# coroa/tmhpvsim

Hardware: AMD Instinct MI355X
Metric: simulated chain-seconds/sec (node) at 1/2/4/8 GPUs + % HBM roofline (higher is better)
Workload: dtype fp32

## Files before the change

### tmhpvsim_amd/csrc/tmh_engine.hip

```cpp
#include <hip/hip_runtime.h>

#include <algorithm>
#include <climits>
#include <cmath>
#include <cstdarg>
#include <cstdio>
#include <cstdlib>
#include <cstring>
#include <string>
#include <type_traits>
#include <utility>
#include <vector>

#include "tmh_math.h"
#include "tmh_model.h"
#include "tmhpvsim.h"

using namespace tmh;
static_assert(OUT_ANY == TMH_OUT_ANY && OUT_TRACE3 == TMH_OUT_TRACE3 && OUT_STATS == TMH_OUT_STATS &&
                  OUT_SERIES == TMH_OUT_SERIES && OUT_INTERVALS == TMH_OUT_INTERVALS &&
                  OUT_REGISTERS == TMH_OUT_REGISTERS && OUT_DEMAND == TMH_OUT_DEMAND && OUT_STORAGE == TMH_OUT_STORAGE,
              "expansion variants: tmh_model.h and include/tmhpvsim.h agree");

namespace {
// ... 101 lines not shown
    ch.pos = st.pos[c];
    ch.status = st.status[c];
    ch.ncalls = st.ncalls[c];
    ch.t1 = ceil_thr(ch.cl);
    ch.t2 = ceil_thr(ch.cl + ch.clr);
}

__device__ __forceinline__ void store_chain(const StateView& st, uint32_t c, const Chain& ch)
{
#pragma unroll
    for (int k = 0; k < 6; ++k) {
        st.sb[k][c] = ch.s.b[k];
        st.sa[k][c] = ch.s.a[k];
    }
    st.cl[c] = ch.cl;
    st.clr[c] = ch.clr;
    st.mstate[c] = ch.mstate;
    st.sec[c] = ch.sec;
    st.L[c] = ch.L;
    st.pos[c] = ch.pos;
    st.status[c] = ch.status;
    st.ncalls[c] = ch.ncalls;
}

constexpr int INIT_SLOT = CAP - 12;

__device__ __forceinline__ void init_cc_pair(const KParams& kp, uint32_t c, const double* u, double& b, double& a)
{
    Chain ch;
    ch.mstate = 1.0;
    b = draw_cc(kp, gid(kp.ids, c), ch, u[0]);
    a = draw_cc(kp, gid(kp.ids, c), ch, u[1]);
}

__global__ __launch_bounds__(256, BUILD_WAVES) void init_variates_kernel(KParams kp, StateView st, uint64_t chain0, uint32_t n,
                                                            double hf)
{
    const uint32_t c = blockIdx.x * blockDim.x + threadIdx.x;
    const int j = 2 + (int)blockIdx.y;
    if (c >= n) return;
    const uint64_t chain = chain0 + gid(kp.ids, c);
    const U4 blk = keyed_block(kp.seed, chain, 0, TAG_INIT, (uint32_t)(j >> 1));
    const double u = (j & 1) ? u52(blk.z, blk.w) : u52(blk.x, blk.y);
    double v;
    if (j <= 3) {
        v = normal(u, 0.99, 0.08);
    } else if (j >= 10) {
        v = 2.14 * gammaincinv(2.69, u);
    } else {
        const U4 b0 = keyed_block(kp.seed, chain, 0, TAG_INIT, 0);
        const double u01[2] = {u52(b0.x, b0.y), u52(b0.z, b0.w)};
        double ccb, cca;
        init_cc_pair(kp, c, u01, ccb, cca);
        const double cc = interp(ccb, cca, hf);
        if (j <= 5) {
            v = cc < 6.0 / 8 ? normal(u, 0.6784, 0.2046) : (cc < 7.0 / 8 ? NAN : gammaincinv(3.5624, u) * 0.0867 + 0.0);
        } else {
            v = j <= 7 ? scaled_noise(kp, u, 0.01, 0.003, cc) : scaled_noise(kp, u, 0.001, 0.0015, cc);
        }
    }
    sig_c(st, c)[INIT_SLOT + j] = v;
}

template <int RNG>
__global__ __launch_bounds__(256, BUILD_WAVES) void init_kernel(KParams kp, StateView st, uint64_t chain0, uint32_t n,
                                                   double hf, InjView inj)
{
    const uint32_t c = blockIdx.x * blockDim.x + threadIdx.x;
    if (c >= n) return;
    Chain ch;
    for (int k = 0; k < 6; ++k) ch.s.b[k] = ch.s.a[k] = NAN;
    ch.cl = ch.clr = NAN;
    ch.mstate = 1.0;
    ch.sec = 0;
    ch.L = 0;
    ch.t1 = ch.t2 = 0;
    ch.pos = 0;
    ch.status = 0;
    ch.ncalls = 0;
    Draw<RNG> dr;
    if constexpr (RNG == TMH_RNG_KEYED) {
        dr.seed = kp.seed;
        dr.chain = chain0 + gid(kp.ids, c);
    } else {
        dr.u = inj.u + (size_t)c * inj.stride;
        dr.len = inj.len;
    }
    const double* pre = sig_c(st, c) + INIT_SLOT;
    double u[12];
    if constexpr (RNG == TMH_RNG_KEYED) {
        dr.two(ch, 0, TAG_INIT, 0, u[0], u[1]);
    } else {
        for (int d = 0; d < 12; d += 2) dr.two(ch, 0, TAG_INIT, (uint32_t)(d >> 1), u[d], u[d + 1]);
    }
    ch.s.b[S_CC] = draw_cc(kp, gid(kp.ids, c), ch, u[0]);
    ch.s.a[S_CC] = draw_cc(kp, gid(kp.ids, c), ch, u[1]);
    if constexpr (RNG == TMH_RNG_KEYED) {
        ch.s.b[S_CLEAR_DAY] = pre[2];
        ch.s.a[S_CLEAR_DAY] = pre[3];
    } else {
        ch.s.b[S_CLEAR_DAY] = normal(u[2], 0.99, 0.08);
        ch.s.a[S_CLEAR_DAY] = normal(u[3], 0.99, 0.08);
    }
    bool name_error = false;
    for (int j = 0; j < 2; ++j) {
        const double cc = interp(ch.s.b[S_CC], ch.s.a[S_CC], hf);
        double v;
        if (cc < 6.0 / 8) v = RNG == TMH_RNG_KEYED ? pre[4 + j] : normal(u[4 + j], 0.6784, 0.2046);
        else if (cc < 7.0 / 8) {
            name_error = true;
            break;
        } else v = RNG == TMH_RNG_KEYED ? pre[4 + j] : gammaincinv(3.5624, u[4 + j]) * 0.0867 + 0.0;
        if (j == 0) ch.s.b[S_CLOUDY_HOUR] = v;
        else ch.s.a[S_CLOUDY_HOUR] = v;
    }
    if (name_error) {
        if constexpr (RNG == TMH_RNG_INJECTED) ch.pos = ch.pos < 4 ? ch.pos : 4;
        ch.status = TMH_CHAIN_NAMEERROR_INIT;
        store_chain(st, c, ch);
        return;
    }
    if constexpr (RNG == TMH_RNG_KEYED) {
        ch.s.b[S_CLOUDY_NOISE] = pre[6];
        ch.s.a[S_CLOUDY_NOISE] = pre[7];
        ch.s.b[S_CLEAR_NOISE] = pre[8];
        ch.s.a[S_CLEAR_NOISE] = pre[9];
        ch.s.b[S_WS] = pre[10];
        ch.s.a[S_WS] = pre[11];
    } else {
        const double cch = interp(ch.s.b[S_CC], ch.s.a[S_CC], hf);
        ch.s.b[S_CLOUDY_NOISE] = scaled_noise(kp, u[6], 0.01, 0.003, cch);
        ch.s.a[S_CLOUDY_NOISE] = scaled_noise(kp, u[7], 0.01, 0.003, cch);
        ch.s.b[S_CLEAR_NOISE] = scaled_noise(kp, u[8], 0.001, 0.0015, cch);
        ch.s.a[S_CLEAR_NOISE] = scaled_noise(kp, u[9], 0.001, 0.0015, cch);
        ch.s.b[S_WS] = 2.14 * gammaincinv(2.69, u[10]);
        ch.s.a[S_WS] = 2.14 * gammaincinv(2.69, u[11]);
    }
    const double h0 = interp(ch.s.b[S_CC], ch.s.a[S_CC], 0.0);
    const double h = 0.95 < h0 ? 0.95 : h0;
    const double ws = interp(ch.s.b[S_WS], ch.s.a[S_WS], 0.0);
    double* sc = sig_c(st, c);
    double* sl = sig_l(st, c);
    const uint32_t f = next_cloud_fresh<RNG>(kp, sc, sl, ch, dr, h, ws, TAG_INIT_CLOUD);
    if (!f) {
        const double us = dr.one(ch, 0, TAG_INIT_SEC, 0, 0);
        ch.sec = (int32_t)((ch.cl + ch.clr) * us);
    }
    if (f && !ch.status) ch.status = f;
    store_chain(st, c, ch);
    st.fn[0][c] = make_float2((float)ch.s.b[S_CLOUDY_NOISE], (float)ch.s.a[S_CLOUDY_NOISE]);
    st.fn[1][c] = make_float2((float)ch.s.b[S_CLEAR_NOISE], (float)ch.s.a[S_CLEAR_NOISE]);
}

__global__ __launch_bounds__(256, BUILD_WAVES) void geom_kernel(GParams gp, int64_t step0, uint32_t n, double* tab64,
                                                   float* tab32, double* sun)
{
    const uint32_t j = blockIdx.x * blockDim.x + threadIdx.x;
    if (j >= n) return;
    const tmh_clock& ck = gp.clock;
    const int64_t s = step0 + j;
    const int64_t lt = local_at(ck, s), lp = local_at(ck, s > 0 ? s - 1 : 0);
    const int64_t dn = floordiv(lt, 86400), dp = floordiv(lp, 86400);
    const int64_t sod = lt - dn * 86400, sodp = lp - dp * 86400;
    const int hour = (int)(sod / 3600), minute = (int)((sod / 60) % 60), second = (int)(sod % 60);
    const int hourp = (int)(sodp / 3600), minutep = (int)((sodp / 60) % 60);
    double g[ROW];
    for (int i = 0; i < ROW; ++i) g[i] = 0.0;
    clock_fractions(hour, minute, second, g[G_MINF], g[G_HOURF], g[G_DAYF]);
    uint32_t fl = 0;
    if (dn != dp) fl |= FL_DAY;
    if (hour != hourp) fl |= FL_HOUR;
    if (minute != minutep) fl |= FL_MIN;
    int doy, leap;
    civil_doy(dn, doy, leap);
    double sn[SUN_W];
    sun_at(ck.utc0 + s, doy, leap, gp.linke, sn);
    {
        const uint32_t jb = j / BLOCK_STEPS * BLOCK_STEPS;
        double sb[SUN_W];
        if (jb == j) {
            sb[SUN_MIN] = sn[SUN_MIN];
            sb[SUN_EOT] = sn[SUN_EOT];
        } else {
            const int64_t ltb = local_at(ck, step0 + jb);
            int doyb, leapb;
            civil_doy(floordiv(ltb, 86400), doyb, leapb);
            sun_at(ck.utc0 + step0 + jb, doyb, leapb, nullptr, sb);
        }
        const double dh = rad(((sn[SUN_MIN] + sn[SUN_EOT]) - (sb[SUN_MIN] + sb[SUN_EOT])) / 4.0);
        sincos(dh, &sn[SUN_SDH], &sn[SUN_CDH]);
    }
    for (int i = 0; i < SUN_W; ++i) sun[(size_t)j * SUN_W + i] = sn[i];
    site_geom<true>(site_k(gp.site), sn, sn[SUN_TL], gp.module, g);
    if (g[G_GHICS] == 0.0) fl |= FL_NIGHT;
    if (g[G_DISCOK] != 0.0) fl |= FL_DISCOK;
    g[G_FLAGS] = (double)fl;
    double* o64 = tab64 + (size_t)j * ROW;
    for (int i = 0; i < ROW; ++i) o64[i] = g[i];
    table_row32(g, fl, tab32 + (size_t)j * ROW32);
}

__global__ __launch_bounds__(256) void group_kind_kernel(int64_t step0, uint32_t n, float* tab32, double* tab64)
{
    static_assert(BLOCK_STEPS == 128, "a block's 32 groups are the 32 lanes of a half-wave");
    const uint32_t g = blockIdx.x * blockDim.x + threadIdx.x, j = 4 * g;
    uint32_t f[4] = {0u, 0u, 0u, 0u}, k = 0;
    if ((step0 & 3) == 0 && j + 3 < n) {
        uint32_t ev = 0, all = ~0u;
#pragma unroll
        for (int q = 0; q < 4; ++q) {
            f[q] = __float_as_uint(tab32[(size_t)(j + q) * ROW32 + G_FLAGS + G32]);
            all &= f[q];
            if (q > 0) ev |= f[q] & (FL_DAY | FL_HOUR | FL_MIN);
        }
        const uint32_t anyn = (f[0] | f[1] | f[2] | f[3]) & FL_NIGHT;
        if (!ev && (all & FL_NIGHT)) k = FL_G_NIGHT;
        else if (!ev && !anyn && (all & FL_DISCOK)) k = FL_G_DAY;
    }
    const uint64_t ng = __builtin_amdgcn_ballot_w64(k == FL_G_NIGHT);
    const uint32_t half = (threadIdx.x & 32u) ? (uint32_t)(ng >> 32) : (uint32_t)ng;
    if ((threadIdx.x & 31u) == 0 && half == ~0u) k |= FL_B_NIGHT;
    if (k) {
        tab32[(size_t)j * ROW32 + G_FLAGS + G32] = __uint_as_float(f[0] | k);
        tab64[(size_t)j * ROW + G_FLAGS] = (double)(f[0] | k);
    }
}

__global__ __launch_bounds__(1024) void block_order_kernel(const float* __restrict__ tab32, int64_t step0, uint32_t n,
                                                           uint32_t* __restrict__ perm)
{
    __shared__ uint32_t cnt[1024];
    const uint32_t t = threadIdx.x, nb = (n + BLOCK_STEPS - 1) / BLOCK_STEPS;
    const uint32_t chunk = (nb + 1023) / 1024, lo = min(t * chunk, nb), hi = min(lo + chunk, nb);
    auto night = [&](uint32_t b) {
        return (__float_as_uint(tab32[(size_t)b * BLOCK_STEPS * ROW32 + G_FLAGS + G32]) & FL_B_NIGHT) != 0;
    };
    uint32_t d = 0;
    for (uint32_t b = lo; b < hi; ++b) d += night(b) ? 0u : 1u;
    cnt[t] = d;
    __syncthreads();
    for (uint32_t off = 1; off < 1024; off <<= 1) {
        const uint32_t v = t >= off ? cnt[t - off] : 0;
        __syncthreads();
        cnt[t] += v;
        __syncthreads();
    }
    const uint32_t nday = cnt[1023];
    uint32_t od = cnt[t] - d, on = nday + (lo - od);
    for (uint32_t b = lo; b < hi; ++b) perm[night(b) ? on++ : od++] = b;
}

__global__ __launch_bounds__(1024) void events_kernel(const float* __restrict__ tab32, int64_t step0, uint32_t n,
                                                      int64_t utc0, int2* events, uint32_t cap, uint32_t* n_events)
{
    __shared__ uint32_t cnt[1024];
    const uint32_t t = threadIdx.x;
    const int64_t first = (60 - (((utc0 + step0) % 60) + 60) % 60) % 60;
    const uint32_t ncand = first < (int64_t)n ? (uint32_t)((n - 1 - first) / 60 + 1) : 0;
    const uint32_t chunk = (ncand + 1023) / 1024;
    const uint32_t lo = t * chunk, hi = min(lo + chunk, ncand);
    uint32_t c = 0;
    for (uint32_t q = lo; q < hi; ++q) {
        const uint64_t j = (uint64_t)(first + 60 * (int64_t)q);
        if (__float_as_uint(tab32[j * ROW32 + G_FLAGS + G32]) & (FL_DAY | FL_HOUR)) ++c;
    }
    cnt[t] = c;
    __syncthreads();
    for (uint32_t off = 1; off < 1024; off <<= 1) {
        const uint32_t v = t >= off ? cnt[t - off] : 0;
        __syncthreads();
        cnt[t] += v;
        __syncthreads();
    }
    uint32_t o = cnt[t] - c;
    for (uint32_t q = lo; q < hi; ++q) {
        const uint64_t j = (uint64_t)(first + 60 * (int64_t)q);
        const uint32_t fl = __float_as_uint(tab32[j * ROW32 + G_FLAGS + G32]) & (FL_DAY | FL_HOUR);
        if (fl) {
            if (o < cap) events[o] = make_int2((int)(step0 + (int64_t)j), (int)fl);
            ++o;
        }
    }
    if (t == 1023) *n_events = cnt[1023];
}

__device__ __forceinline__ uint32_t ev_cap_dev(uint32_t n_steps) { return n_steps / 3600 + 16; }

__host__ __device__ __forceinline__ int64_t first_minute(int64_t utc0, int64_t W0)
{
    return (60 - (((utc0 + W0) % 60) + 60) % 60) % 60;
}
inline int64_t first_minute_host(int64_t utc0, int64_t W0) { return first_minute(utc0, W0); }

__device__ BlockDesc desc_for(int64_t step0, uint32_t n, int64_t utc0, const int2* __restrict__ events, int ne,
                              int64_t p)
{
    BlockDesc d{-1, -1, -1, -1, -1, -1, 0, -1};
    {
        const int64_t lo = step0 > 1 ? step0 : 1;
        const int64_t fm = first_minute(utc0, step0);
        const int64_t m0 = p - (((utc0 + p) % 60) + 60) % 60;
        if (m0 >= lo) d.q0 = (int32_t)((m0 - step0 - fm) / 60);
        if (m0 - 60 >= lo) d.q1 = (int32_t)((m0 - 60 - step0 - fm) / 60);
        int a = 0, z = ne;
        while (a < z) {
            const int mid = (a + z) / 2;
            if (events[mid].x <= p) a = mid + 1;
            else z = mid;
        }
        d.evi = a;
        int nh = 0, ncd = 0;
        for (int i = a - 1; i >= 0 && (nh < 3 || ncd < 2); --i) {
            const int fl = events[i].y;
            if (fl & FL_HOUR) {
                if (nh == 0) d.h0 = i;
                else if (nh == 1) d.h1 = i;
                else if (nh == 2) d.h2 = i;
                ++nh;
                if (ncd < 2) {
                    if (ncd == 0) d.cd0 = 2 * i + 1;
                    else d.cd1 = 2 * i + 1;
                    ++ncd;
                }
            }
            if ((fl & FL_DAY) && ncd < 2) {
                if (ncd == 0) d.cd0 = 2 * i;
                else d.cd1 = 2 * i;
                ++ncd;
            }
        }
    }
    return d;
}

__device__ __forceinline__ BlockDesc desc_advance(BlockDesc d, int64_t step0, int64_t utc0,
                                                  const int2* __restrict__ events, int ne, int64_t p)
{
    int i = d.evi;
    for (; i < ne && (int64_t)events[i].x <= p; ++i) {
        const int fl = events[i].y;
        if (fl & FL_DAY) {
            d.cd1 = d.cd0;
            d.cd0 = 2 * i;
        }
        if (fl & FL_HOUR) {
            d.h2 = d.h1;
            d.h1 = d.h0;
            d.h0 = i;
            d.cd1 = d.cd0;
            d.cd0 = 2 * i + 1;
        }
    }
    d.evi = i;
    const int64_t lo = step0 > 1 ? step0 : 1, fm = first_minute(utc0, step0);
    const int64_t m0 = p - (((utc0 + p) % 60) + 60) % 60;
    d.q0 = m0 >= lo ? (int32_t)((m0 - step0 - fm) / 60) : -1;
    d.q1 = m0 - 60 >= lo ? (int32_t)((m0 - 60 - step0 - fm) / 60) : -1;
    return d;
}

__global__ __launch_bounds__(256) void desc_kernel(int64_t step0, uint32_t n, int64_t utc0,
                                                   const int2* __restrict__ events,
                                                   const uint32_t* __restrict__ n_events, BlockDesc* desc,
                                                   uint32_t nblk)
{
    const uint32_t b = blockIdx.x * blockDim.x + threadIdx.x;
    if (b > nblk) return;
    const int64_t jb = min((int64_t)b * BLOCK_STEPS, (int64_t)n);
    desc[b] = jb > 0 ? desc_for(step0, n, utc0, events, (int)min(*n_events, ev_cap_dev(n)), step0 + jb - 1)
                     : BlockDesc{-1, -1, -1, -1, -1, -1, 0, -1};
}

__device__ __forceinline__ int first_t_bin(const KParams& kp, uint32_t c, double& df)
{
    const uint32_t r = gid(kp.ids, c);
    for (int b = 0; b < 6; ++b) {
        const int t = kp.tab && kp.tab_t ? kp.tab_t[(size_t)r * 6 + b] : kp.is_t[b];
        if (t) {
            df = kp.tab ? kp.tab[(size_t)r * 24 + 4 * b + 3] : kp.shapes[b][3];
            return b;
        }
    }
    df = 0.0;
    return -1;
}

__global__ __launch_bounds__(256, BUILD_WAVES) void event_draws_kernel(DrawParams dp, KParams kp, bool mk_pre, uint64_t chain0,
                                                          uint32_t n, uint32_t nsteps, const int2* __restrict__ events,
                                                          const uint32_t* __restrict__ n_events, double* evd,
                                                          uint32_t* identity_order, uint32_t* identity_rank)
{
    const uint32_t c = blockIdx.y * blockDim.x + threadIdx.x;
    const uint32_t e = blockIdx.x;
    if (identity_order && e == 0 && c < n) {
        identity_order[c] = c;
        identity_rank[c] = c;
    }
    if (c >= n || e >= min(*n_events, ev_cap_dev(nsteps))) return;
    const uint64_t chain = chain0 + gid(dp.ids, c), step = (uint64_t)events[e].x;
    const int fl = events[e].y;
    double* o = evd + (size_t)e * 4 * n + c;
    if (fl & FL_DAY) {
        const U4 u = keyed_block(dp.seed, chain, step, TAG_BOUNDARY, 0);
        o[2 * (size_t)n] = normal(u52(u.x, u.y), 0.99, 0.08);
        o[(size_t)n] = 2.14 * gammaincinv(2.69, u52(u.z, u.w));
    }
    if (fl & FL_HOUR) {
        const U4 u = keyed_block(dp.seed, chain, step, TAG_BOUNDARY, 1);
        if (!dp.markov) {
            o[0] = cc_faithful(dp, gid(dp.ids, c), u52(u.x, u.y));
        } else if (mk_pre) {
            double df;
            const int tb = first_t_bin(kp, c, df);
            o[0] = tb >= 0 ? stdtrit(df, u52(u.x, u.y)) : 0.0;
        }
        o[3 * (size_t)n] = normal(u52(u.z, u.w), 0.99, 0.08);
    }
}

constexpr int MK_BLOCK = 256;
__global__ __launch_bounds__(MK_BLOCK) void markov_cc_kernel(KParams kp, bool mk_pre, StateView st, uint64_t chain0, uint32_t n,
                                                        uint32_t nsteps, const int2* __restrict__ events,
                                                        const uint32_t* __restrict__ n_events, double* evd,
                                                        PrevView prev)
{
    __shared__ double2 tab_s[MK_BLOCK * 12];
    __shared__ int32_t tabt_s[MK_BLOCK * 6];
    const uint32_t cb0 = blockIdx.x * MK_BLOCK;
    const uint32_t nb = min((uint32_t)MK_BLOCK, n - cb0);
    if (kp.tab && !kp.ids) {
        const double2* src = reinterpret_cast<const double2*>(kp.tab + (size_t)cb0 * 24);
        for (uint32_t i = threadIdx.x; i < nb * 12; i += MK_BLOCK) tab_s[i] = src[i];
        for (uint32_t i = threadIdx.x; i < nb * 6; i += MK_BLOCK)
            tabt_s[i] = kp.tab_t ? kp.tab_t[(size_t)cb0 * 6 + i] : kp.is_t[i % 6];
    } else if (kp.tab) {
        for (uint32_t i = threadIdx.x; i < nb * 12; i += MK_BLOCK) {
            const uint32_t g = kp.ids[cb0 + i / 12];
            tab_s[i] = reinterpret_cast<const double2*>(kp.tab + (size_t)g * 24)[i % 12];
        }
        for (uint32_t i = threadIdx.x; i < nb * 6; i += MK_BLOCK)
            tabt_s[i] = kp.tab_t ? kp.tab_t[(size_t)kp.ids[cb0 + i / 6] * 6 + i % 6] : kp.is_t[i % 6];
    }
    __syncthreads();
    const uint32_t c = cb0 + threadIdx.x;
    if (c >= n) return;
    const uint64_t chain = chain0 + gid(kp.ids, c);
    const uint32_t ne = min(*n_events, ev_cap_dev(nsteps));
    const double* row = kp.tab ? reinterpret_cast<const double*>(tab_s) + threadIdx.x * 24 : nullptr;
    const int32_t* rowt = tabt_s + threadIdx.x * 6;
    double state = prev.status ? prev.end_p1[(size_t)n + c] : st.mstate[c];
    int tb = -1;
    if (mk_pre)
        for (int b = 5; b >= 0; --b)
            if (row ? rowt[b] : kp.is_t[b]) tb = b;
    for (uint32_t e = 0; e < ne; ++e) {
        const int2 ev = events[e];
        if (!(ev.y & FL_HOUR)) continue;
        const double qt = mk_pre ? evd[(size_t)e * 4 * n + c] : 0.0;
        const U4 u4 = keyed_block(kp.seed, chain, (uint64_t)ev.x, TAG_BOUNDARY, 1);
        const double u = u52(u4.x, u4.y);
        int bin = 5;
#pragma unroll
        for (int k = 4; k >= 0; --k) bin = kp.edges[k] < state ? bin : k;
        double loc, scale, kappa, df;
        int is_t;
        if (row) {
            const double* sh = row + 4 * bin;
            loc = sh[0];
            scale = sh[1];
            kappa = sh[2];
            df = sh[3];
            is_t = rowt[bin];
        } else {
            loc = kp.shapes[bin][0];
            scale = kp.shapes[bin][1];
            kappa = kp.shapes[bin][2];
            df = kp.shapes[bin][3];
            is_t = kp.is_t[bin];
        }
        const bool t_here = is_t && bin != tb;
        const uint64_t tl = __builtin_amdgcn_ballot_w64(t_here);
        const uint64_t al = __builtin_amdgcn_ballot_w64(is_t == 0);
        double v = is_t ? qt : 0.0;
        if (tl && t_here) v = stdtrit(df, u);
        if (al && !is_t) v = al_ppf(u, kappa);
        v = v * scale + loc;
        const double x = state + v;
        state = x < 0.0 ? 0.0 : (x > 1.0 ? 1.0 : x);
        evd[(size_t)e * 4 * n + c] = state;
    }
}

template <typename R>
__device__ __forceinline__ void minute_draws(const DrawParams& dp, uint64_t chain, int64_t step, double cc,
                                             double& cloudy, double& clear)
{
    const U4 u = keyed_block(dp.seed, chain, (uint64_t)step, TAG_BOUNDARY, 2);
    if constexpr (sizeof(R) == 8) {
        cloudy = minute_noise<R>(u52(u.x, u.y), 0.01, 0.003, cc, dp.sqrt09);
        clear = minute_noise<R>(u52(u.z, u.w), 0.001, 0.0015, cc, dp.sqrt09);
    } else {
        cloudy = minute_noise_fast(u52(u.x, u.y), 0.01, 0.003, cc, dp.sqrt09);
        clear = minute_noise_fast(u52(u.z, u.w), 0.001, 0.0015, cc, dp.sqrt09);
    }
}

__device__ __forceinline__ double minute_cc(const StateView& st, const PrevView& prev, const SegView& sg, uint32_t n,
                                            uint32_t c, int64_t W0, int64_t jm, const int2* __restrict__ events, int ne,
                                            const double* __restrict__ tab64)
{
    const int64_t step = W0 + jm;
    int lo = 0, hi = ne;
    while (lo < hi) {
        const int mid = (lo + hi) >> 1;
        if ((int64_t)events[mid].x <= step) lo = mid + 1;
        else hi = mid;
    }
    const int h0 = lo - 1, h1 = lo - 2;
    const double* evd = sg.evd;
    const double sb = prev.status ? prev.end_p1[c] : st.sb[S_CC][c];
    const double sa = prev.status ? prev.end_p1[(size_t)n + c] : st.sa[S_CC][c];
    double pb, pa;
    if (h0 < 0) {
        pb = sb;
// ... 3266 lines not shown
    eng->walk_lanes = lanes;
    return TMH_OK;
}

int tmh_set_walk_order(struct tmh_engine* eng, int on)
{
    if (!eng) return fail(TMH_E_INVAL, "NULL engine");
    eng->walk_order = on != 0;
    return TMH_OK;
}

int tmh_stream_create_cus(uint32_t cu_first, uint32_t cu_count, void** stream)
{
    if (!stream) return fail(TMH_E_INVAL, "NULL stream out");
    *stream = nullptr;
    hipStream_t s = nullptr;
    if (cu_count == 0) {
        if (int rc = hip_check(hipStreamCreateWithFlags(&s, hipStreamNonBlocking), "hipStreamCreate")) return rc;
        *stream = s;
        return TMH_OK;
    }
    int dev = 0, ncu = 0;
    if (int rc = hip_check(hipGetDevice(&dev), "hipGetDevice")) return rc;
    if (int rc = hip_check(hipDeviceGetAttribute(&ncu, hipDeviceAttributeMultiprocessorCount, dev), "CU count")) return rc;
    if ((uint64_t)cu_first + cu_count > (uint64_t)ncu)
        return fail(TMH_E_INVAL, "CU range %u + %u past the device's %d CUs", cu_first, cu_count, ncu);
    std::vector<uint32_t> mask((ncu + 31) / 32, 0u);
    for (uint32_t i = cu_first; i < cu_first + cu_count; ++i) mask[i >> 5] |= 1u << (i & 31);
    if (int rc = hip_check(hipExtStreamCreateWithCUMask(&s, (uint32_t)mask.size(), mask.data()), "hipExtStreamCreateWithCUMask"))
        return rc;
    *stream = s;
    return TMH_OK;
}

int tmh_stream_destroy(void* stream)
{
    if (!stream) return TMH_OK;
    return hip_check(hipStreamDestroy((hipStream_t)stream), "hipStreamDestroy");
}

int tmh_set_chain_ids(struct tmh_engine* eng, const uint32_t* ids, uint32_t n_full)
{
    if (!eng) return fail(TMH_E_INVAL, "NULL engine");
    if (ids && n_full == 0) return fail(TMH_E_INVAL, "chain ids with n_full 0");
    eng->kp.ids = eng->dp.ids = ids;
    eng->kp.ids_n = ids ? n_full : 0;
    return TMH_OK;
}

int tmh_live_chains(struct tmh_engine* eng, const void* state, uint32_t n_chains, const uint32_t* ids_in,
                    uint32_t* ids_out, uint32_t* n_live, void* stream)
{
    if (!eng || !state || !ids_out || !n_live) return fail(TMH_E_INVAL, "NULL engine/state/ids_out/n_live");
    if (int rc = hip_check(hipSetDevice(eng->device), "hipSetDevice")) return rc;
    hipLaunchKernelGGL(live_chains_kernel, dim3(1), dim3(1024), 0, (hipStream_t)stream,
                       make_view(const_cast<void*>(state), n_chains), n_chains, ids_in, ids_out, n_live);
    return hip_check(hipGetLastError(), "live_chains_kernel launch");
}

int tmh_state_move(struct tmh_engine* eng, const void* src, uint32_t n_src, void* dst, uint32_t n_dst,
                   const uint32_t* map, const uint32_t* count, uint32_t cap, int scatter, void* stream)
{
    if (!eng || !src || !dst || !map || !count) return fail(TMH_E_INVAL, "NULL engine/src/dst/map/count");
    if (cap > (scatter ? n_src : n_dst)) return fail(TMH_E_INVAL, "cap %u exceeds the moved-to/from slots", cap);
    if (cap == 0) return TMH_OK;
    if (int rc = hip_check(hipSetDevice(eng->device), "hipSetDevice")) return rc;
    hipLaunchKernelGGL(state_move_kernel, dim3((cap + 255) / 256), dim3(256), 0, (hipStream_t)stream,
                       make_view(const_cast<void*>(src), n_src), make_view(dst, n_dst), map, count, cap, scatter);
    return hip_check(hipGetLastError(), "state_move_kernel launch");
}

int tmh_test_set_segment_capacity(uint32_t cap, uint32_t pool_chunks)
{
    if (cap % 16) return fail(TMH_E_INVAL, "segment capacity %u is not a multiple of 16", cap);
    g_cap_override = cap;
    g_pool_override = pool_chunks;
    return TMH_OK;
}

int64_t tmh_test_guard_records(const struct tmh_engine* eng, const void* scratch, uint32_t n_chains, uint32_t n_steps)
{
    if (!eng || !scratch || n_chains == 0 || n_steps == 0) return fail(TMH_E_INVAL, "NULL engine/scratch or empty window");
    if (eng->path != TMH_PATH_TIME_PARALLEL) return fail(TMH_E_INVAL, "guard records: the time-parallel path only");
    if (int rc = hip_check(hipSetDevice(eng->device), "hipSetDevice")) return rc;
    SegView sg;
    scratch_layout(n_chains, n_steps, const_cast<void*>(scratch), &sg, tmh_engine_scratch_rbytes(eng));
    uint32_t k = 0;
    if (int rc = hip_check(hipMemcpy(&k, sg.nfix, sizeof k, hipMemcpyDeviceToHost), "guard records copy")) return rc;
    return (int64_t)k;
}

int tmh_profile_enable(struct tmh_engine* eng, int on)
{
    if (!eng) return fail(TMH_E_INVAL, "NULL engine");
    eng->profiling = on != 0;
    return TMH_OK;
}

int tmh_profile_read(struct tmh_engine* eng, int kernel, double* total_ms, int* launches)
{
    if (!eng || !total_ms || kernel < 0 || kernel >= TMH_K_COUNT) return fail(TMH_E_INVAL, "bad profile_read args");
    if (int rc = hip_check(hipSetDevice(eng->device), "hipSetDevice")) return rc;
    double t = 0.0;
    int n = 0;
    for (auto& p : eng->prof[kernel]) {
        if (int rc = hip_check(hipEventSynchronize(p.second), "hipEventSynchronize")) return rc;
        float ms = 0.f;
        if (int rc = hip_check(hipEventElapsedTime(&ms, p.first, p.second), "hipEventElapsedTime")) return rc;
        t += ms;
        ++n;
        eng->pool.push_back(p.first);
        eng->pool.push_back(p.second);
    }
    eng->prof[kernel].clear();
    *total_ms = t;
    if (launches) *launches = n;
    return TMH_OK;
}

int tmh_init(struct tmh_engine* eng, void* state, uint64_t chain0, uint32_t n_chains, const tmh_ustream* inj,
             void* stream)
{
    if (!eng || !state) return fail(TMH_E_INVAL, "NULL engine/state");
    if (n_chains == 0) return TMH_OK;
    if (eng->kp.rng_mode == TMH_RNG_INJECTED && (!inj || !inj->u || inj->stride < inj->len))
        return fail(TMH_E_INVAL, "injected mode needs a stream with stride >= len");
    if (int rc = check_tables(eng, n_chains)) return rc;
    if (int rc = hip_check(hipSetDevice(eng->device), "hipSetDevice")) return rc;
    int64_t sod = eng->local_step0 % 86400;
    if (sod < 0) sod += 86400;
    const double hf = ((int)((sod / 60) % 60) + (int)(sod % 60) / 60.0) / 60.0;
    StateView v = make_view(state, n_chains);
    InjView iv{inj ? inj->u : nullptr, inj ? inj->stride : 0, inj ? inj->len : 0};
    dim3 grid((n_chains + 255) / 256), block(256);
    hipStream_t s = (hipStream_t)stream;
    if (eng->kp.rng_mode == TMH_RNG_KEYED)
        hipLaunchKernelGGL(init_variates_kernel, dim3(grid.x, 10), block, 0, s, eng->kp, v, chain0, n_chains, hf);
    with_value<TMH_RNG_KEYED, TMH_RNG_INJECTED>(eng->kp.rng_mode, [&](auto rng) {
        hipLaunchKernelGGL(init_kernel<decltype(rng)::value>, grid, block, 0, s, eng->kp, v, chain0, n_chains, hf, iv);
    });
    return hip_check(hipGetLastError(), "init_kernel launch");
}

int tmh_plan(struct tmh_engine* eng, int64_t step0, uint32_t n_steps, void* plan, void* stream)
{
    if (!eng || !plan) return fail(TMH_E_INVAL, "NULL engine/plan");
    if (n_steps == 0) return TMH_OK;
    if (step0 < 0 || step0 + (int64_t)n_steps > (int64_t)INT_MAX - (1 << 20))
        return fail(TMH_E_INVAL, "step window [%lld, +%u) outside [0, 2^31 - 2^20)", (long long)step0, n_steps);
    if (int rc = hip_check(hipSetDevice(eng->device), "hipSetDevice")) return rc;
    PlanView pv;
    plan_layout(n_steps, plan, &pv);
    hipStream_t s = (hipStream_t)stream;
    hipLaunchKernelGGL(geom_kernel, dim3((n_steps + 255) / 256), dim3(256), 0, s, eng->gp, step0, n_steps, pv.tab64,
                       pv.tab32, pv.sun);
    hipLaunchKernelGGL(group_kind_kernel, dim3((n_steps / 4 + 255) / 256 + 1), dim3(256), 0, s, step0, n_steps, pv.tab32,
                       pv.tab64);
    if (eng->cost_order)
        hipLaunchKernelGGL(block_order_kernel, dim3(1), dim3(1024), 0, s, pv.tab32, step0, n_steps, pv.bperm);
    hipLaunchKernelGGL(events_kernel, dim3(1), dim3(1024), 0, s, pv.tab32, step0, n_steps, eng->gp.clock.utc0,
                       pv.events, ev_cap(n_steps), pv.n_events);
    const uint32_t nb = nblk_of(n_steps);
    hipLaunchKernelGGL(desc_kernel, dim3((nb + 1 + 255) / 256), dim3(256), 0, s, step0, n_steps, eng->gp.clock.utc0,
                       pv.events, pv.n_events, pv.desc, nb);
    return hip_check(hipGetLastError(), "plan kernels launch");
}

enum { PH_DRAWS = 1, PH_SEGMENTS = 4, PH_WALK = PH_DRAWS | PH_SEGMENTS, PH_EXPAND = 2, PH_COMMIT = 8, PH_ALL = 15 };

struct StepCtx {
    tmh_engine* eng;
    hipStream_t s;
    uint64_t chain0;
    uint32_t n_chains;
    int64_t step0;
    uint32_t n_steps;
    PrevView prev;
    StateView v;
    PlanView pv;
    SegView sg;
    InjView iv;
    TraceView tv;
    StatsView sv;
    SeriesView sev;
    IntervalsView ivv;
    bool f64() const { return eng->kp.precision == TMH_FP64; }
    bool series() const { return eng->has_series; }
    int table() const { return eng->table_kind(); }
    uint32_t cb() const { return (n_chains + 255) / 256; }
    int64_t utc0() const { return eng->gp.clock.utc0; }
};

static int phase_draws(const StepCtx& c)
{
    tmh_engine* const eng = c.eng;
    hipStream_t s = c.s;
    const dim3 cbs(c.cb()), t256(256);
    const bool mk_pre = eng->dp.markov && c.n_chains <= eng->mk_pre_max;
    hipLaunchKernelGGL(event_draws_kernel, dim3(c.sg.evcap, c.cb()), t256, 0, s, eng->dp, eng->kp, mk_pre, c.chain0,
                       c.n_chains, c.n_steps, c.pv.events, c.pv.n_events, c.sg.evd,
                       eng->walk_order ? nullptr : c.sg.order, eng->walk_order ? nullptr : c.sg.rank);
    if (eng->dp.markov)
        hipLaunchKernelGGL(markov_cc_kernel, cbs, t256, 0, s, eng->kp, mk_pre, c.v, c.chain0, c.n_chains, c.n_steps,
                           c.pv.events, c.pv.n_events, c.sg.evd, c.prev);
    if (eng->walk_order) {
        const uint32_t tiles = (c.n_chains + ORDER_TILE - 1) / ORDER_TILE;
        if (tiles <= WALK_RANK_TILES)
            hipLaunchKernelGGL(walk_rank_kernel, dim3(tiles * (ORDER_TILE / ORDER_EPB)), t256, 0, s, c.v, c.n_chains,
                               c.sg, c.prev);
        else
            hipLaunchKernelGGL(walk_order_kernel, dim3(tiles), dim3(1024), 0, s, c.v, c.n_chains, c.sg, c.prev);
    }
    hipEvent_t t_cand = eng->mark(s);
    {
        const int64_t fmh = first_minute_host(c.utc0(), c.step0);
        const uint32_t nm = fmh < (int64_t)c.n_steps ? (uint32_t)((c.n_steps - 1 - fmh) / 60 + 1) : 0;
        const uint32_t ny = c.sg.kcap + nm;
        const dim3 grid(c.cb(), std::min(ny, 65535u));
        const BlockDesc* de = c.pv.desc + nblk_of(c.n_steps);
        with_real(c.f64(), [&](auto r) {
            hipLaunchKernelGGL(draws_tail_kernel<decltype(r)>, grid, t256, 0, s, eng->dp, c.v, c.chain0, c.n_chains,
                               c.step0, c.n_steps, fmh, ny, c.pv.tab64, c.pv.events, c.pv.n_events, de, c.sg, c.prev);
        });
    }
    eng->close(TMH_K_CANDIDATES, t_cand, s);
    return hip_check(hipGetLastError(), "draws kernels launch");
}

static int phase_segments(const StepCtx& c)
{
    tmh_engine* const eng = c.eng;
    hipStream_t s = c.s;
    hipEvent_t t_seg = eng->mark(s);
    const uint32_t rows = (uint32_t)(((uint64_t)c.n_chains + eng->walk_cpr - 1) / eng->walk_cpr);
    const uint32_t G = eng->walk_lanes ? eng->walk_lanes : (c.n_chains > WALK_AUTO_SMALL ? 4u : 16u);
    const uint32_t gpw = 16;
    const dim3 wg((rows + gpw - 1) / gpw), wt(gpw * G);
    const size_t wlds = gpw * WALK_CAND * sizeof(double);
    const bool q = rows < c.n_chains;
    const int mode = q ? 1 : (G == 8 && rows >= eng->walk_tp_rows) ? 2 : 0;
    with_value<4, 8, 16>((int)G, [&](auto lanes) {
        with_value<0, 1, 2>(mode, [&](auto m) {
            constexpr int GG = decltype(lanes)::value, M = decltype(m)::value;
            constexpr bool Q = M == 1, TP = M == 2;
            if constexpr (!TP || GG == 8)
                hipLaunchKernelGGL((segments_kernel<Q, GG, TP>), wg, wt, wlds, s, eng->dp, c.v, c.chain0, c.n_chains,
                                   c.step0, c.n_steps, eng->gp.clock, c.pv.events, c.pv.n_events, c.sg, c.prev);
        });
    });
    hipLaunchKernelGGL(overflow_settle_kernel, dim3(c.cb()), dim3(256), 0, s, c.n_chains, c.sg);
    hipLaunchKernelGGL(block_rec_kernel, dim3(c.cb(), (c.sg.nblk + BREC_G - 1) / BREC_G), dim3(256), 0, s, c.n_chains,
                       c.step0, c.sg);
    eng->close(TMH_K_SEGMENTS, t_seg, s);
    return hip_check(hipGetLastError(), "segments kernel launch");
}

static int phase_expand(const StepCtx& c)
{
    tmh_engine* const eng = c.eng;
    const TraceView& tv = c.tv;
    const StatsView& sv = c.sv;
    hipEvent_t t_exp = eng->mark(c.s);
    const bool f64 = c.f64(), sites = eng->kp.sites != nullptr, no_stats = !sv.hist && !sv.acc;
    const int table = c.table();
    int out = table != TBL_KINDS ? TABLE_KINDS[table].out
              : c.series() ? OUT_SERIES
              : (no_stats && tv.pv && tv.meter && tv.residual && !tv.csi && !tv.covered) ? OUT_TRACE3
                    : (!tv.pv && !tv.meter && !tv.residual && !tv.csi && !tv.covered) ? OUT_STATS
                                                                                      : OUT_ANY;
    if (out == OUT_TRACE3 && tv.ld * (f64 ? 8u : 4u) * BLOCK_STEPS >= (1ull << 31))
        return fail(TMH_E_INVAL, "trace ld %llu too large (a 128-step block of rows must stay under 2 GiB)",
                    (unsigned long long)tv.ld);
    if (sites && out == OUT_TRACE3) out = OUT_ANY;
    auto launch = [&](auto r, auto okind, auto st, const auto& view, const StatsView& sv) {
        using R = decltype(r);
        constexpr int O = decltype(okind)::value;
        constexpr bool S = decltype(st)::value;
        constexpr uint32_t wg = exp_wg<R, O, S>();
        constexpr bool pack = exp_hist_pack<R, O, S>();
        const size_t bins = sv.n_bins, lds = pack ? (bins + 1) / 2 * 4 : bins * 4;
        hipLaunchKernelGGL((expand_kernel<R, O, S>), dim3(c.sg.nblk, (c.n_chains + wg - 1) / wg), dim3(wg), lds, c.s,
                           eng->kp, eng->dp, c.v,
                           c.chain0, c.n_chains, c.step0, c.n_steps, c.utc0(), c.pv.tab64, c.pv.tab32, c.pv.sun,
                           c.pv.events, c.pv.n_events, c.pv.desc, c.sg, view, sv, eng->cost_order ? c.pv.bperm : nullptr);
    };
    const bool b64 = !f64 && sv.hist && sv.bin64;
    with_real(f64, [&](auto r) {
        with_value<0, 1>(sites, [&](auto st) {
            constexpr bool F32 = sizeof(r) == 4, S = decltype(st)::value;
            auto traces = [&](auto okind) { launch(r, okind, st, tv, sv); };
            auto ivl = [&](auto okind) { launch(r, okind, st, c.ivv, sv); };
            if (table == TBL_STORAGE) {
                if constexpr (!F32) {
                    const tmh_storage& sb = eng->storage;
                    const StorageView stv{c.ivv, reinterpret_cast<long long*>(sb.work), (long long)sb.capacity,
                                          (int)sb.p_charge, (int)sb.p_discharge};
                    hipEvent_t t = eng->mark(c.s);
                    launch(r, std::integral_constant<int, OUT_STORAGE | OUT_MAP>{}, st, stv, StatsView{});
                    eng->close(TMH_K_STORAGE_MAP, t, c.s);
                    t = eng->mark(c.s);
                    hipLaunchKernelGGL(storage_scan_kernel, dim3(c.cb()), dim3(256), 0, c.s, stv.work,
                                       reinterpret_cast<long long*>(sb.soc), eng->kp.ids, c.n_chains, c.sg.nblk);
                    eng->close(TMH_K_STORAGE_SCAN, t, c.s);
                    t = eng->mark(c.s);
                    launch(r, std::integral_constant<int, OUT_STORAGE>{}, st, stv, sv);
                    eng->close(TMH_K_STORAGE_REPLAY, t, c.s);
                }
            } else if (table == TBL_BATTERY) {
                if constexpr (!F32) {
                    const tmh_battery& bb = eng->battery;
                    const long long* params = reinterpret_cast<const long long*>(bb.params);
                    const BatteryView btv{StorageView{c.ivv, reinterpret_cast<long long*>(bb.work), 0, 0, 0}, params};
                    hipEvent_t t = eng->mark(c.s);
                    launch(r, std::integral_constant<int, OUT_STORAGE | OUT_LOSSY | OUT_MAP>{}, st, btv, StatsView{});
                    eng->close(TMH_K_STORAGE_MAP, t, c.s);
                    t = eng->mark(c.s);
                    hipLaunchKernelGGL(battery_scan_kernel, dim3(c.cb()), dim3(256), 0, c.s, btv.st.work,
// ... 300 lines not shown
```

Baseline: 292.8 billion.

## Fuse plan geometry, grouping, events and descriptors into one kernel

Replaces the separate geom, group_kind, events and desc launches with a single plan_kernel. Most workgroups compute table rows and derive group and block night flags from shared memory instead of re-reading tab32. A few leading workgroups recompute the clock flags directly to build the event list, then fill the block descriptors. This removes several launches and dependent global round-trips, and skips writing the sun table when no sites use it. In exchange, each event workgroup redundantly rebuilds the full event list and writes identical values to the same buffer, which relies on benign races. The night-block detection now spans two waves through shared memory.

```diff
diff --git a/tmhpvsim_amd/csrc/tmh_engine.hip b/tmhpvsim_amd/csrc/tmh_engine.hip
--- a/tmhpvsim_amd/csrc/tmh_engine.hip
+++ b/tmhpvsim_amd/csrc/tmh_engine.hip
@@ -277,25 +277,33 @@
     st.fn[1][c] = make_float2((float)ch.s.b[S_CLEAR_NOISE], (float)ch.s.a[S_CLEAR_NOISE]);
 }
 
-__global__ __launch_bounds__(256, BUILD_WAVES) void geom_kernel(GParams gp, int64_t step0, uint32_t n, double* tab64,
-                                                   float* tab32, double* sun)
-{
-    const uint32_t j = blockIdx.x * blockDim.x + threadIdx.x;
-    if (j >= n) return;
-    const tmh_clock& ck = gp.clock;
-    const int64_t s = step0 + j;
+__device__ __forceinline__ uint32_t clock_flags(const tmh_clock& ck, int64_t s, int64_t& dn, int& hour, int& minute,
+                                                int& second)
+{
     const int64_t lt = local_at(ck, s), lp = local_at(ck, s > 0 ? s - 1 : 0);
-    const int64_t dn = floordiv(lt, 86400), dp = floordiv(lp, 86400);
+    dn = floordiv(lt, 86400);
+    const int64_t dp = floordiv(lp, 86400);
     const int64_t sod = lt - dn * 86400, sodp = lp - dp * 86400;
-    const int hour = (int)(sod / 3600), minute = (int)((sod / 60) % 60), second = (int)(sod % 60);
+    hour = (int)(sod / 3600), minute = (int)((sod / 60) % 60), second = (int)(sod % 60);
     const int hourp = (int)(sodp / 3600), minutep = (int)((sodp / 60) % 60);
-    double g[ROW];
-    for (int i = 0; i < ROW; ++i) g[i] = 0.0;
-    clock_fractions(hour, minute, second, g[G_MINF], g[G_HOURF], g[G_DAYF]);
     uint32_t fl = 0;
     if (dn != dp) fl |= FL_DAY;
     if (hour != hourp) fl |= FL_HOUR;
     if (minute != minutep) fl |= FL_MIN;
+    return fl;
+}
+
+__device__ __forceinline__ uint32_t plan_row(const GParams& gp, int64_t step0, uint32_t j, double* tab64, float* tab32,
+                                             double* sun)
+{
+    const tmh_clock& ck = gp.clock;
+    const int64_t s = step0 + j;
+    int64_t dn;
+    int hour, minute, second;
+    uint32_t fl = clock_flags(ck, s, dn, hour, minute, second);
+    double g[ROW];
+    for (int i = 0; i < ROW; ++i) g[i] = 0.0;
+    clock_fractions(hour, minute, second, g[G_MINF], g[G_HOURF], g[G_DAYF]);
     int doy, leap;
     civil_doy(dn, doy, leap);
     double sn[SUN_W];
@@ -315,7 +323,8 @@
         const double dh = rad(((sn[SUN_MIN] + sn[SUN_EOT]) - (sb[SUN_MIN] + sb[SUN_EOT])) / 4.0);
         sincos(dh, &sn[SUN_SDH], &sn[SUN_CDH]);
     }
-    for (int i = 0; i < SUN_W; ++i) sun[(size_t)j * SUN_W + i] = sn[i];
+    if (sun)
+        for (int i = 0; i < SUN_W; ++i) sun[(size_t)j * SUN_W + i] = sn[i];
     site_geom<true>(site_k(gp.site), sn, sn[SUN_TL], gp.module, g);
     if (g[G_GHICS] == 0.0) fl |= FL_NIGHT;
     if (g[G_DISCOK] != 0.0) fl |= FL_DISCOK;
@@ -323,31 +332,39 @@
     double* o64 = tab64 + (size_t)j * ROW;
     for (int i = 0; i < ROW; ++i) o64[i] = g[i];
     table_row32(g, fl, tab32 + (size_t)j * ROW32);
-}
-
-__global__ __launch_bounds__(256) void group_kind_kernel(int64_t step0, uint32_t n, float* tab32, double* tab64)
-{
-    static_assert(BLOCK_STEPS == 128, "a block's 32 groups are the 32 lanes of a half-wave");
-    const uint32_t g = blockIdx.x * blockDim.x + threadIdx.x, j = 4 * g;
-    uint32_t f[4] = {0u, 0u, 0u, 0u}, k = 0;
-    if ((step0 & 3) == 0 && j + 3 < n) {
-        uint32_t ev = 0, all = ~0u;
+    return fl;
+}
+
+__device__ __forceinline__ void plan_rows(const GParams& gp, int64_t step0, uint32_t n, uint32_t j0, double* tab64,
+                                          float* tab32, double* sun)
+{
+    static_assert(BLOCK_STEPS == 128, "a block's 32 groups are the first-row lanes of two waves");
+    __shared__ uint32_t fls[256];
+    __shared__ uint32_t wnight[4];
+    const uint32_t t = threadIdx.x, j = j0 + t;
+    fls[t] = j < n ? plan_row(gp, step0, j, tab64, tab32, sun) : 0u;
+    __syncthreads();
+    uint32_t f0 = 0, k = 0;
+    if ((t & 3u) == 0 && (step0 & 3) == 0 && j + 3 < n) {
+        uint32_t f[4], ev = 0, all = ~0u;
 #pragma unroll
         for (int q = 0; q < 4; ++q) {
-            f[q] = __float_as_uint(tab32[(size_t)(j + q) * ROW32 + G_FLAGS + G32]);
+            f[q] = fls[t + q];
             all &= f[q];
             if (q > 0) ev |= f[q] & (FL_DAY | FL_HOUR | FL_MIN);
         }
         const uint32_t anyn = (f[0] | f[1] | f[2] | f[3]) & FL_NIGHT;
         if (!ev && (all & FL_NIGHT)) k = FL_G_NIGHT;
         else if (!ev && !anyn && (all & FL_DISCOK)) k = FL_G_DAY;
+        f0 = f[0];
     }
     const uint64_t ng = __builtin_amdgcn_ballot_w64(k == FL_G_NIGHT);
-    const uint32_t half = (threadIdx.x & 32u) ? (uint32_t)(ng >> 32) : (uint32_t)ng;
-    if ((threadIdx.x & 31u) == 0 && half == ~0u) k |= FL_B_NIGHT;
+    if ((t & 63u) == 0) wnight[t >> 6] = ng == 0x1111111111111111ull;
+    __syncthreads();
+    if ((t & 127u) == 0 && wnight[t >> 6] && wnight[(t >> 6) + 1]) k |= FL_B_NIGHT;
     if (k) {
-        tab32[(size_t)j * ROW32 + G_FLAGS + G32] = __uint_as_float(f[0] | k);
-        tab64[(size_t)j * ROW + G_FLAGS] = (double)(f[0] | k);
+        tab32[(size_t)j * ROW32 + G_FLAGS + G32] = __uint_as_float(f0 | k);
+        tab64[(size_t)j * ROW + G_FLAGS] = (double)(f0 | k);
     }
 }
 
@@ -375,23 +392,28 @@
     for (uint32_t b = lo; b < hi; ++b) perm[night(b) ? on++ : od++] = b;
 }
 
-__global__ __launch_bounds__(1024) void events_kernel(const float* __restrict__ tab32, int64_t step0, uint32_t n,
-                                                      int64_t utc0, int2* events, uint32_t cap, uint32_t* n_events)
-{
-    __shared__ uint32_t cnt[1024];
-    const uint32_t t = threadIdx.x;
-    const int64_t first = (60 - (((utc0 + step0) % 60) + 60) % 60) % 60;
+__device__ __forceinline__ uint32_t ev_cap_dev(uint32_t n_steps) { return n_steps / 3600 + 16; }
+
+__device__ __forceinline__ uint32_t plan_events(const tmh_clock& ck, int64_t step0, uint32_t n, int2* events,
+                                                uint32_t* n_events)
+{
+    __shared__ uint32_t cnt[256];
+    const uint32_t t = threadIdx.x, cap = ev_cap_dev(n);
+    const int64_t first = (60 - (((ck.utc0 + step0) % 60) + 60) % 60) % 60;
     const uint32_t ncand = first < (int64_t)n ? (uint32_t)((n - 1 - first) / 60 + 1) : 0;
-    const uint32_t chunk = (ncand + 1023) / 1024;
-    const uint32_t lo = t * chunk, hi = min(lo + chunk, ncand);
+    const uint32_t chunk = (ncand + 255) / 256;
+    const uint32_t lo = min(t * chunk, ncand), hi = min(lo + chunk, ncand);
+    auto flags = [&](uint32_t q) {
+        int64_t dn;
+        int hour, minute, second;
+        return clock_flags(ck, step0 + first + 60 * (int64_t)q, dn, hour, minute, second) & (FL_DAY | FL_HOUR);
+    };
     uint32_t c = 0;
-    for (uint32_t q = lo; q < hi; ++q) {
-        const uint64_t j = (uint64_t)(first + 60 * (int64_t)q);
-        if (__float_as_uint(tab32[j * ROW32 + G_FLAGS + G32]) & (FL_DAY | FL_HOUR)) ++c;
-    }
+    for (uint32_t q = lo; q < hi; ++q)
+        if (flags(q)) ++c;
     cnt[t] = c;
     __syncthreads();
-    for (uint32_t off = 1; off < 1024; off <<= 1) {
+    for (uint32_t off = 1; off < 256; off <<= 1) {
         const uint32_t v = t >= off ? cnt[t - off] : 0;
         __syncthreads();
         cnt[t] += v;
@@ -399,17 +421,16 @@
     }
     uint32_t o = cnt[t] - c;
     for (uint32_t q = lo; q < hi; ++q) {
-        const uint64_t j = (uint64_t)(first + 60 * (int64_t)q);
-        const uint32_t fl = __float_as_uint(tab32[j * ROW32 + G_FLAGS + G32]) & (FL_DAY | FL_HOUR);
+        const uint32_t fl = flags(q);
         if (fl) {
-            if (o < cap) events[o] = make_int2((int)(step0 + (int64_t)j), (int)fl);
+            if (o < cap) events[o] = make_int2((int)(step0 + first + 60 * (int64_t)q), (int)fl);
             ++o;
         }
     }
-    if (t == 1023) *n_events = cnt[1023];
-}
-
-__device__ __forceinline__ uint32_t ev_cap_dev(uint32_t n_steps) { return n_steps / 3600 + 16; }
+    const uint32_t ne = cnt[255];
+    if (t == 255) *n_events = ne;
+    return ne;
+}
 
 __host__ __device__ __forceinline__ int64_t first_minute(int64_t utc0, int64_t W0)
 {
@@ -484,17 +505,24 @@
     return d;
 }
 
-__global__ __launch_bounds__(256) void desc_kernel(int64_t step0, uint32_t n, int64_t utc0,
-                                                   const int2* __restrict__ events,
-                                                   const uint32_t* __restrict__ n_events, BlockDesc* desc,
-                                                   uint32_t nblk)
-{
-    const uint32_t b = blockIdx.x * blockDim.x + threadIdx.x;
-    if (b > nblk) return;
-    const int64_t jb = min((int64_t)b * BLOCK_STEPS, (int64_t)n);
-    desc[b] = jb > 0 ? desc_for(step0, n, utc0, events, (int)min(*n_events, ev_cap_dev(n)), step0 + jb - 1)
-                     : BlockDesc{-1, -1, -1, -1, -1, -1, 0, -1};
-}
+__global__ __launch_bounds__(256, BUILD_WAVES) void plan_kernel(GParams gp, int64_t step0, uint32_t n, uint32_t ev_wgs,
+                                                                double* tab64, float* tab32, double* sun, int2* events,
+                                                                uint32_t* n_events, BlockDesc* desc, uint32_t nblk)
+{
+    if (blockIdx.x >= ev_wgs) {
+        plan_rows(gp, step0, n, (blockIdx.x - ev_wgs) * 256u, tab64, tab32, sun);
+        return;
+    }
+    const int ne = (int)min(plan_events(gp.clock, step0, n, events, n_events), ev_cap_dev(n));
+    __syncthreads();
+    for (uint32_t b = blockIdx.x * 256u + threadIdx.x; b <= nblk; b += ev_wgs * 256u) {
+        const int64_t jb = min((int64_t)b * BLOCK_STEPS, (int64_t)n);
+        desc[b] = jb > 0 ? desc_for(step0, n, gp.clock.utc0, events, ne, step0 + jb - 1)
+                         : BlockDesc{-1, -1, -1, -1, -1, -1, 0, -1};
+    }
+}
+
+inline uint32_t plan_ev_wgs(uint32_t nblk) { return std::min((nblk + 1 + 1023) / 1024, 8u); }
 
 __device__ __forceinline__ int first_t_bin(const KParams& kp, uint32_t c, double& df)
 {
@@ -4067,17 +4095,11 @@
     PlanView pv;
     plan_layout(n_steps, plan, &pv);
     hipStream_t s = (hipStream_t)stream;
-    hipLaunchKernelGGL(geom_kernel, dim3((n_steps + 255) / 256), dim3(256), 0, s, eng->gp, step0, n_steps, pv.tab64,
-                       pv.tab32, pv.sun);
-    hipLaunchKernelGGL(group_kind_kernel, dim3((n_steps / 4 + 255) / 256 + 1), dim3(256), 0, s, step0, n_steps, pv.tab32,
-                       pv.tab64);
+    const uint32_t nb = nblk_of(n_steps), ev_wgs = plan_ev_wgs(nb);
+    hipLaunchKernelGGL(plan_kernel, dim3(ev_wgs + (n_steps + 255) / 256), dim3(256), 0, s, eng->gp, step0, n_steps, ev_wgs,
+                       pv.tab64, pv.tab32, eng->kp.sites ? pv.sun : nullptr, pv.events, pv.n_events, pv.desc, nb);
     if (eng->cost_order)
         hipLaunchKernelGGL(block_order_kernel, dim3(1), dim3(1024), 0, s, pv.tab32, step0, n_steps, pv.bperm);
-    hipLaunchKernelGGL(events_kernel, dim3(1), dim3(1024), 0, s, pv.tab32, step0, n_steps, eng->gp.clock.utc0,
-                       pv.events, ev_cap(n_steps), pv.n_events);
-    const uint32_t nb = nblk_of(n_steps);
-    hipLaunchKernelGGL(desc_kernel, dim3((nb + 1 + 255) / 256), dim3(256), 0, s, step0, n_steps, eng->gp.clock.utc0,
-                       pv.events, pv.n_events, pv.desc, nb);
     return hip_check(hipGetLastError(), "plan kernels launch");
 }
 
```

Measured after the change: 292.4 billion. Within noise of the previous version (-0.1%).
